# andrewdalpino/UltraZoom

Hardware: AMD Instinct MI355X
Metric: upscaled MPix/sec, MewZoom-4X 1080p bf16 batched inference (higher is better)
Workload: dtype bf16; 1 GPU; MewZoom-4X 96ch/40L bf16, 16 x 1080x1920 -> 4320x7680 per GPU; global_batch=16, parallelism=batch-sharded x1, images_in_flight=0

## Files before the change

ultrazoom_amd/csrc/mz_mix16.h:

```cpp
#pragma once
#include "mz_device.h"

namespace mz {

__device__ __forceinline__ void mix_blend_pair(float& o0, float& o1, const float b0, const float b1, const float x0, const float x1,
                                               const float z0, const float z1, const float inv_s) {
    float d0, d1;
    asm("v_mul_f32 %0, 0xbfb8aa3b, %4\n\t"
        "v_mul_f32 %1, 0xbfb8aa3b, %5\n\t"
        "v_exp_f32 %0, %0\n\t"
        "v_exp_f32 %1, %1\n\t"
        "v_fma_f32 %0, %0, %10, %10\n\t"
        "v_fma_f32 %1, %1, %10, %10\n\t"
        "v_rcp_f32 %0, %0\n\t"
        "v_rcp_f32 %1, %1\n\t"
        "v_sub_f32 %2, %8, %6\n\t"
        "v_sub_f32 %3, %9, %7\n\t"
        "v_fma_f32 %0, %0, %2, %6\n\t"
        "v_fma_f32 %1, %1, %3, %7"
        : "=&v"(o0), "=&v"(o1), "=&v"(d0), "=&v"(d1)
        : "v"(b0), "v"(b1), "v"(x0), "v"(x1), "v"(z0), "v"(z1), "s"(inv_s));
}

struct MixFrag {
    u32x4 w[3][2];
};
template <class TT, int G>
__device__ __forceinline__ void mix16_group(f32x4 (&acc)[2][12], MixFrag& f, const u32x4 (&xb)[2], uint32_t b_addr) {
    constexpr int n = G % 6, wp = G % 3;
    if constexpr (G + 2 < 24) {
        f.w[(G + 2) % 3][0] = lds_read128<(((G + 2) / 6) * 12 + 2 * ((G + 2) % 6)) * 1024>(b_addr);
        f.w[(G + 2) % 3][1] = lds_read128<(((G + 2) / 6) * 12 + 2 * ((G + 2) % 6) + 1) * 1024>(b_addr);
    }
    __builtin_amdgcn_sched_barrier(0);
    constexpr int p0 = G & 1, p1 = p0 ^ 1;
    mma16<TT>(acc[p0][2 * n], f.w[wp][0], xb[p0]);
    mma16<TT>(acc[p0][2 * n + 1], f.w[wp][1], xb[p0]);
    mma16<TT>(acc[p1][2 * n + 1], f.w[wp][1], xb[p1]);
    mma16<TT>(acc[p1][2 * n], f.w[wp][0], xb[p1]);
    __builtin_amdgcn_sched_barrier(0);
    if constexpr (G + 1 < 24) wait_w16<(G + 2 < 24 ? 2 : 0)>(f.w[(G + 1) % 3][0], f.w[(G + 1) % 3][1]);
}
template <class TT, int KS> __device__ __forceinline__ void mix16_kstep(f32x4 (&acc)[2][12], MixFrag& f, const u32x4 (&xb)[2], uint32_t b_addr) {
    mix16_group<TT, KS * 6 + 0>(acc, f, xb, b_addr);
    mix16_group<TT, KS * 6 + 1>(acc, f, xb, b_addr);
    mix16_group<TT, KS * 6 + 2>(acc, f, xb, b_addr);
    mix16_group<TT, KS * 6 + 3>(acc, f, xb, b_addr);
    mix16_group<TT, KS * 6 + 4>(acc, f, xb, b_addr);
    mix16_group<TT, KS * 6 + 5>(acc, f, xb, b_addr);
}

template <class TT>
__global__ __launch_bounds__(576) void mix16_kernel(const ConvArgs a) {
    constexpr int STAGE = 4 * 12 * 1024;
    extern __shared__ __attribute__((aligned(16))) char smem[];
    const int tid = threadIdx.x;
    const int lane = tid & 63;
    const int w = __builtin_amdgcn_readfirstlane(tid >> 6);
    int mtile, ntile;
    if (!map_tile(a, mtile, ntile)) return;
    const int nsteps = a.nchunks16;
    const int nstages = nsteps >> 2;

    if (w == 8) {
        const char* src = (const char*)a.wpk16 + (size_t)ntile * nsteps * (12 * 1024) + lane * 16;
        auto issue = [&](int st) __attribute__((always_inline)) {
            char* dst = smem + (st & 1) * STAGE;
#pragma unroll
            for (int j = 0; j < 48; ++j) glds16(src + (size_t)st * STAGE + j * 1024, dst + j * 1024);
        };
        issue(0);
        for (int st = 0; st < nstages; ++st) {
            wait_vmcnt<0>();
            __builtin_amdgcn_s_barrier();
            if (st + 1 < nstages) issue(st + 1);
        }
        return;
    }

    const int g = lane >> 4, c = lane & 15;
    const long long hw = (long long)a.Ho * a.Wo;
    const long long M = (long long)a.B * hw;
    const int half_steps = nsteps >> 1;
    const uint32_t tensor_bytes = (uint32_t)((long long)a.B * a.p0 * hw * 16);
    const __amdgpu_buffer_rsrc_t xr = __builtin_amdgcn_make_buffer_rsrc((void*)a.in0, 0, (int)tensor_bytes, 0x00020000);
    const __amdgpu_buffer_rsrc_t zr = __builtin_amdgcn_make_buffer_rsrc((void*)a.in1, 0, (int)tensor_bytes, 0x00020000);
    uint32_t voff[2];
    uint32_t vpix[2];
#pragma unroll
    for (int pf = 0; pf < 2; ++pf) {
        const long long m = (long long)mtile * 256 + 32 * w + 16 * pf + c;
        const bool in = m < M;
        const long long mm = in ? m : 0;
        const int bimg = (int)(mm / hw);
        const long long pix = mm - (long long)bimg * hw;
        vpix[pf] = in ? (uint32_t)((((long long)bimg * a.p0) * hw + pix) * 16) : 0xffffffffu;
        voff[pf] = in ? (uint32_t)((((long long)bimg * a.p0 + g) * hw + pix) * 16) : 0xffffffffu;
    }
    const uint32_t step_bytes = (uint32_t)(4 * hw * 16);
    auto load_b = [&](int ks, u32x4 (&xb)[2]) __attribute__((always_inline)) {
        const bool isz = ks >= half_steps;
        const int kk = ks >= nsteps ? 0 : (isz ? ks - half_steps : ks);
        const int so = __builtin_amdgcn_readfirstlane((int)(kk * step_bytes));
#pragma unroll
        for (int pf = 0; pf < 2; ++pf)
            xb[pf] = isz ? __builtin_amdgcn_raw_buffer_load_b128(zr, (int)voff[pf], so, 0)
                         : __builtin_amdgcn_raw_buffer_load_b128(xr, (int)voff[pf], so, 0);
    };
    f32x4 acc[2][12];
#pragma unroll
    for (int pf = 0; pf < 2; ++pf)
#pragma unroll
        for (int nf = 0; nf < 12; ++nf) acc[pf][nf] = f32x4{0.f, 0.f, 0.f, 0.f};
    const uint32_t lds_base = (uint32_t)(uintptr_t)(__attribute__((address_space(3))) char*)smem;
    const uint32_t b_lane = lds_base + lane * 16;
    u32x4 xb0[2], xb1[2], xb2[2];
    load_b(0, xb0);
    load_b(1, xb1);
    MixFrag f;
    auto stage_head = [&](uint32_t b_addr) __attribute__((always_inline)) {
        __builtin_amdgcn_s_barrier();
        f.w[0][0] = lds_read128<0>(b_addr);
        f.w[0][1] = lds_read128<1024>(b_addr);
        f.w[1][0] = lds_read128<2048>(b_addr);
        f.w[1][1] = lds_read128<3072>(b_addr);
        wait_w16<2>(f.w[0][0], f.w[0][1]);
    };
    for (int st = 0; st < nstages; st += 3) {
        const int ks = 4 * st;
        uint32_t b_addr = b_lane + (st & 1) * STAGE;
        stage_head(b_addr);
        load_b(ks + 2, xb2);  mix16_kstep<TT, 0>(acc, f, xb0, b_addr);
        load_b(ks + 3, xb0);  mix16_kstep<TT, 1>(acc, f, xb1, b_addr);
        load_b(ks + 4, xb1);  mix16_kstep<TT, 2>(acc, f, xb2, b_addr);
        load_b(ks + 5, xb2);  mix16_kstep<TT, 3>(acc, f, xb0, b_addr);
        b_addr = b_lane + ((st + 1) & 1) * STAGE;
        stage_head(b_addr);
        load_b(ks + 6, xb0);  mix16_kstep<TT, 0>(acc, f, xb1, b_addr);
        load_b(ks + 7, xb1);  mix16_kstep<TT, 1>(acc, f, xb2, b_addr);
        load_b(ks + 8, xb2);  mix16_kstep<TT, 2>(acc, f, xb0, b_addr);
        load_b(ks + 9, xb0);  mix16_kstep<TT, 3>(acc, f, xb1, b_addr);
        b_addr = b_lane + (st & 1) * STAGE;
        stage_head(b_addr);
        load_b(ks + 10, xb1); mix16_kstep<TT, 0>(acc, f, xb2, b_addr);
        load_b(ks + 11, xb2); mix16_kstep<TT, 1>(acc, f, xb0, b_addr);
        load_b(ks + 12, xb0); mix16_kstep<TT, 2>(acc, f, xb1, b_addr);
        load_b(ks + 13, xb1); mix16_kstep<TT, 3>(acc, f, xb2, b_addr);
    }
    const int nbase = ntile * 192;
    const uint32_t plane_bytes = (uint32_t)(hw * 16);
    typedef uint32_t u32x2_ __attribute__((ext_vector_type(2)));
    struct XZ { u32x2_ x[2], z[2]; };
    auto request = [&](int i, XZ& q) __attribute__((always_inline)) {
        const int pf = i / 6, n = i - 6 * pf;
        const bool in = vpix[pf] != 0xffffffffu;
#pragma unroll
        for (int k = 0; k < 2; ++k) {
            const int nf = 2 * n + k;
            const int plane = (nbase >> 3) + 2 * nf + (g >> 1);
            const uint32_t off = in ? vpix[pf] + (uint32_t)plane * plane_bytes + (g & 1) * 8 : 0xffffffffu;
            q.x[k] = __builtin_amdgcn_raw_buffer_load_b64(xr, (int)off, 0, 0);
            q.z[k] = __builtin_amdgcn_raw_buffer_load_b64(zr, (int)off, 0, 0);
        }
    };
    auto finish = [&](int i, const XZ& q) __attribute__((always_inline)) {
        const int pf = i / 6, n = i - 6 * pf;
        const bool in = vpix[pf] != 0xffffffffu;
        float v[8];
#pragma unroll
        for (int k = 0; k < 2; ++k) {
            const int nf = 2 * n + k;
            float xv[4], zv[4];
            unpack2<TT>(q.x[k][0], xv[0], xv[1]); unpack2<TT>(q.x[k][1], xv[2], xv[3]);
            unpack2<TT>(q.z[k][0], zv[0], zv[1]); unpack2<TT>(q.z[k][1], zv[2], zv[3]);
            float o0, o1, o2, o3;
            mix_blend_pair(o0, o1, acc[pf][nf][0], acc[pf][nf][1], xv[0], xv[1], zv[0], zv[1], a.inv_mix_scale);
            mix_blend_pair(o2, o3, acc[pf][nf][2], acc[pf][nf][3], xv[2], xv[3], zv[2], zv[3], a.inv_mix_scale);
            acc[pf][nf] = f32x4{o0, o1, o2, o3};
        }
#pragma unroll
        for (int j = 0; j < 4; ++j) {
            const float ea = acc[pf][2 * n][j], eb = acc[pf][2 * n + 1][j];
            const auto sw = __builtin_amdgcn_permlane16_swap(__builtin_bit_cast(uint32_t, ea), __builtin_bit_cast(uint32_t, eb), false, false);
            const uint32_t s0 = sw[0], s1 = sw[1];
            v[j] = __builtin_bit_cast(float, s0);
            v[4 + j] = __builtin_bit_cast(float, s1);
        }
        const int cu = 2 * (2 * n + (g & 1)) + (g >> 1);
        if (in) st_unit<TT>((char*)a.out + vpix[pf] + (long long)((nbase >> 3) + cu) * plane_bytes, v);
    };
    XZ qa, qb;
    request(0, qa);
#pragma unroll
    for (int i = 0; i < 12; i += 2) {
        request(i + 1, qb);
        __builtin_amdgcn_sched_barrier(0);
        finish(i, qa);
        if (i + 2 < 12) request(i + 2, qa);
        __builtin_amdgcn_sched_barrier(0);
        finish(i + 1, qb);
    }
}

template <class TT>
__global__ __launch_bounds__(512) void mix16b_kernel(const ConvArgs a) {
    constexpr int STAGE = 4 * 12 * 1024;
    extern __shared__ __attribute__((aligned(16))) char smem[];
    const int tid = threadIdx.x;
    const int lane = tid & 63;
    const int w = __builtin_amdgcn_readfirstlane(tid >> 6);
    {
        const char* wsrc = (const char*)a.wpk16 + lane * 16 + w * (18 * 1024);
        char* dst = smem + w * (18 * 1024);
#pragma unroll
        for (int j = 0; j < 18; ++j) glds16(wsrc + j * 1024, dst + j * 1024);
    }
    const int g = lane >> 4, c = lane & 15;
    const long long hw = (long long)a.Ho * a.Wo;
    const long long M = (long long)a.B * hw;
    const uint32_t tensor_bytes = (uint32_t)((long long)a.B * a.p0 * hw * 16);
    const __amdgpu_buffer_rsrc_t xr = __builtin_amdgcn_make_buffer_rsrc((void*)a.in0, 0, (int)tensor_bytes, 0x00020000);
    const __amdgpu_buffer_rsrc_t zr = __builtin_amdgcn_make_buffer_rsrc((void*)a.in1, 0, (int)tensor_bytes, 0x00020000);
    const __amdgpu_buffer_rsrc_t orr = __builtin_amdgcn_make_buffer_rsrc((void*)a.out, 0, (int)tensor_bytes, 0x00020000);
    const uint32_t step_bytes = (uint32_t)(4 * hw * 16);
    const float inv_hw = 1.0f / (float)hw;
    const int hwi = (int)hw, Mi = (int)M;
    auto offsets = [&](int u, uint32_t (&vo)[2]) __attribute__((always_inline)) {
#pragma unroll
        for (int pf = 0; pf < 2; ++pf) {
            const int m = u * 32 + 16 * pf + c;
            const bool in = m < Mi;
            const int mm = in ? m : 0;
            int bimg = (int)((float)mm * inv_hw);
            int pix = mm - bimg * hwi;
            if (pix < 0) { bimg -= 1; pix += hwi; }
            if (pix >= hwi) { bimg += 1; pix -= hwi; }
            vo[pf] = in ? ((uint32_t)(bimg * a.p0 + g) * (uint32_t)hwi + (uint32_t)pix) * 16u : 0xffffffffu;
        }
    };
    const int nunits = (Mi + 31) / 32;
    const int stride = (int)gridDim.x * 8;
    int u = (int)blockIdx.x * 8 + w;
    uint32_t voff[2];
    offsets(u, voff);
    u32x4 R[12][2];
#pragma unroll
    for (int i = 0; i < 6; ++i) {
        const int so = __builtin_amdgcn_readfirstlane((int)(i * step_bytes));
#pragma unroll
        for (int pf = 0; pf < 2; ++pf) R[i][pf] = __builtin_amdgcn_raw_buffer_load_b128(xr, (int)voff[pf], so, 0);
    }
#pragma unroll
    for (int i = 0; i < 6; ++i) {
        const int so = __builtin_amdgcn_readfirstlane((int)(i * step_bytes));
#pragma unroll
        for (int pf = 0; pf < 2; ++pf) R[6 + i][pf] = __builtin_amdgcn_raw_buffer_load_b128(zr, (int)voff[pf], so, 0);
    }
    __builtin_amdgcn_sched_barrier(0);
    wait_vmcnt<0>();
    __builtin_amdgcn_s_barrier();
    const uint32_t lds_base = (uint32_t)(uintptr_t)(__attribute__((address_space(3))) char*)smem;
    const uint32_t b_lane = lds_base + lane * 16;
    MixFrag f;
    auto stage_head = [&](uint32_t b_addr) __attribute__((always_inline)) {
        f.w[0][0] = lds_read128<0>(b_addr);
        f.w[0][1] = lds_read128<1024>(b_addr);
        f.w[1][0] = lds_read128<2048>(b_addr);
        f.w[1][1] = lds_read128<3072>(b_addr);
        wait_w16<2>(f.w[0][0], f.w[0][1]);
    };
    while (u < nunits) {
        const int un = u + stride;
        uint32_t vnext[2];
        offsets(un, vnext);
        __builtin_amdgcn_sched_barrier(0);
        f32x4 acc[2][12];
#pragma unroll
        for (int pf = 0; pf < 2; ++pf)
#pragma unroll
            for (int nf = 0; nf < 12; ++nf) acc[pf][nf] = f32x4{0.f, 0.f, 0.f, 0.f};
        stage_head(b_lane);
        mix16_kstep<TT, 0>(acc, f, R[0], b_lane);
        mix16_kstep<TT, 1>(acc, f, R[1], b_lane);
        mix16_kstep<TT, 2>(acc, f, R[2], b_lane);
        mix16_kstep<TT, 3>(acc, f, R[3], b_lane);
        stage_head(b_lane + STAGE);
        mix16_kstep<TT, 0>(acc, f, R[4], b_lane + STAGE);
        mix16_kstep<TT, 1>(acc, f, R[5], b_lane + STAGE);
        mix16_kstep<TT, 2>(acc, f, R[6], b_lane + STAGE);
        mix16_kstep<TT, 3>(acc, f, R[7], b_lane + STAGE);
        stage_head(b_lane + 2 * STAGE);
        mix16_kstep<TT, 0>(acc, f, R[8], b_lane + 2 * STAGE);
        mix16_kstep<TT, 1>(acc, f, R[9], b_lane + 2 * STAGE);
        mix16_kstep<TT, 2>(acc, f, R[10], b_lane + 2 * STAGE);
        mix16_kstep<TT, 3>(acc, f, R[11], b_lane + 2 * STAGE);
#pragma unroll
        for (int m = 0; m < 6; ++m) {
            const int so = __builtin_amdgcn_readfirstlane((int)(m * step_bytes));
#pragma unroll
            for (int pf = 0; pf < 2; ++pf) {
                float v[8];
#pragma unroll
                for (int q = 0; q < 4; ++q) {
                    float xl, xh, zl, zh;
                    unpack2<TT>(R[m][pf][q], xl, xh);
                    unpack2<TT>(R[6 + m][pf][q], zl, zh);
                    mix_blend_pair(v[2 * q], v[2 * q + 1], acc[pf][2 * m + (q >> 1)][2 * (q & 1)], acc[pf][2 * m + (q >> 1)][2 * (q & 1) + 1], xl, xh, zl, zh,
                                   a.inv_mix_scale);
                }
                u32x4 t;
                if constexpr (TT::IS_BF16) {
                    t[0] = pack_bf16(v[0], v[1]); t[1] = pack_bf16(v[2], v[3]); t[2] = pack_bf16(v[4], v[5]); t[3] = pack_bf16(v[6], v[7]);
                } else {
                    t[0] = pack_f16(v[0], v[1]); t[1] = pack_f16(v[2], v[3]); t[2] = pack_f16(v[4], v[5]); t[3] = pack_f16(v[6], v[7]);
                }
                store16_soff(t, orr, (int)voff[pf], so);
            }
#pragma unroll
            for (int pf = 0; pf < 2; ++pf) {
                R[m][pf] = __builtin_amdgcn_raw_buffer_load_b128(xr, (int)vnext[pf], so, 0);
                R[6 + m][pf] = __builtin_amdgcn_raw_buffer_load_b128(zr, (int)vnext[pf], so, 0);
            }
            __builtin_amdgcn_sched_barrier(0);
        }
        u = un;
        voff[0] = vnext[0];
        voff[1] = vnext[1];
    }
}

}
```

ultrazoom_amd/csrc/mz_mix16.hip:

```cpp
#include "mz_mix16.h"

namespace mz {

hipError_t launch_mix16(int dtype, const ConvArgs& a, hipStream_t s) {
    if (!walk_ok(a)) return hipErrorInvalidValue;
    if (a.nchunks16 <= 0 || a.nchunks16 % 12) return hipErrorInvalidValue;
    const size_t lds = 2 * 4 * 12 * 1024;
    switch (dtype) {
        case DT_BF16: return launch_lds<mix16_kernel<TBF16>>(a.grid, 576, lds, a, s);
        case DT_F16: return launch_lds<mix16_kernel<TF16>>(a.grid, 576, lds, a, s);
        default: return hipErrorInvalidValue;
    }
}

hipError_t launch_mix16b(int dtype, const ConvArgs& a, hipStream_t s, int workgroups) {
    if (a.mtiles <= 0 || a.ntiles != 1 || workgroups <= 0) return hipErrorInvalidValue;
    if (a.nchunks16 != 12) return hipErrorInvalidValue;
    const size_t lds = 3 * 4 * 12 * 1024;
    const int grid = a.mtiles < workgroups ? a.mtiles : workgroups;
    switch (dtype) {
        case DT_BF16: return launch_lds<mix16b_kernel<TBF16>>(grid, 512, lds, a, s);
        case DT_F16: return launch_lds<mix16b_kernel<TF16>>(grid, 512, lds, a, s);
        default: return hipErrorInvalidValue;
    }
}

}
```

Before: 708.6 MPix/s.

## Restructure mix16 kernel: drop producer wave, stash operand tiles for epilogue blend

Removes the dedicated producer wave. All 8 compute waves now issue their share of the weight global-to-LDS copies, double-buffered in smaller stages with explicit vmcnt waits. While the main loop streams the x/z activation tiles, the tile this block's output channels correspond to is kept: x goes to an LDS stash and z stays in registers. The epilogue then blends from these instead of re-reading x and z from global memory, and stores with packed 16-byte stores. It uses more LDS, adds registers for the kept z tiles, and adds inline-asm branches and a remapped weight row layout. It also restricts nchunks16 to 12*ntiles.

Result: no change. 710.3 MPix/s (median of 6 runs) (+0.2%).

```diff
diff --git a/ultrazoom_amd/csrc/mz_mix16.h b/ultrazoom_amd/csrc/mz_mix16.h
--- a/ultrazoom_amd/csrc/mz_mix16.h
+++ b/ultrazoom_amd/csrc/mz_mix16.h
@@ -1,5 +1,8 @@
 #pragma once
+#include <type_traits>
+
 #include "mz_device.h"
+#include "mz_mix16_rows.h"
 
 namespace mz {
 
@@ -25,10 +28,10 @@
 struct MixFrag {
     u32x4 w[3][2];
 };
-template <class TT, int G>
+template <class TT, int G, int NG = 24>
 __device__ __forceinline__ void mix16_group(f32x4 (&acc)[2][12], MixFrag& f, const u32x4 (&xb)[2], uint32_t b_addr) {
     constexpr int n = G % 6, wp = G % 3;
-    if constexpr (G + 2 < 24) {
+    if constexpr (G + 2 < NG) {
         f.w[(G + 2) % 3][0] = lds_read128<(((G + 2) / 6) * 12 + 2 * ((G + 2) % 6)) * 1024>(b_addr);
         f.w[(G + 2) % 3][1] = lds_read128<(((G + 2) / 6) * 12 + 2 * ((G + 2) % 6) + 1) * 1024>(b_addr);
     }
@@ -39,20 +42,64 @@
     mma16<TT>(acc[p1][2 * n + 1], f.w[wp][1], xb[p1]);
     mma16<TT>(acc[p1][2 * n], f.w[wp][0], xb[p1]);
     __builtin_amdgcn_sched_barrier(0);
-    if constexpr (G + 1 < 24) wait_w16<(G + 2 < 24 ? 2 : 0)>(f.w[(G + 1) % 3][0], f.w[(G + 1) % 3][1]);
-}
-template <class TT, int KS> __device__ __forceinline__ void mix16_kstep(f32x4 (&acc)[2][12], MixFrag& f, const u32x4 (&xb)[2], uint32_t b_addr) {
-    mix16_group<TT, KS * 6 + 0>(acc, f, xb, b_addr);
-    mix16_group<TT, KS * 6 + 1>(acc, f, xb, b_addr);
-    mix16_group<TT, KS * 6 + 2>(acc, f, xb, b_addr);
-    mix16_group<TT, KS * 6 + 3>(acc, f, xb, b_addr);
-    mix16_group<TT, KS * 6 + 4>(acc, f, xb, b_addr);
-    mix16_group<TT, KS * 6 + 5>(acc, f, xb, b_addr);
+    if constexpr (G + 1 < NG) wait_w16<(G + 2 < NG ? 2 : 0)>(f.w[(G + 1) % 3][0], f.w[(G + 1) % 3][1]);
+}
+template <class TT, int KS, int NG = 24>
+__device__ __forceinline__ void mix16_kstep(f32x4 (&acc)[2][12], MixFrag& f, const u32x4 (&xb)[2], uint32_t b_addr) {
+    mix16_group<TT, KS * 6 + 0, NG>(acc, f, xb, b_addr);
+    mix16_group<TT, KS * 6 + 1, NG>(acc, f, xb, b_addr);
+    mix16_group<TT, KS * 6 + 2, NG>(acc, f, xb, b_addr);
+    mix16_group<TT, KS * 6 + 3, NG>(acc, f, xb, b_addr);
+    mix16_group<TT, KS * 6 + 4, NG>(acc, f, xb, b_addr);
+    mix16_group<TT, KS * 6 + 5, NG>(acc, f, xb, b_addr);
+}
+
+template <int OFF> __device__ __forceinline__ void lds_write128(uint32_t addr, const u32x4& v) {
+    static_assert(OFF >= 0 && OFF < 65536, "ds offset is 16 bits");
+    asm volatile("ds_write_b128 %0, %1 offset:%2" ::"v"(addr), "v"(v), "n"(OFF) : "memory");
+}
+
+__device__ __forceinline__ void keep16_if_eq(u32x4& kept, const u32x4& v, int a, int b) {
+    uint32_t k0 = kept[0], k1 = kept[1], k2 = kept[2], k3 = kept[3];
+    const uint32_t v0 = v[0], v1 = v[1], v2 = v[2], v3 = v[3];
+    asm volatile("s_cmp_lg_u32 %8, %9\n\t"
+                 "s_cbranch_scc1 .Lmix16_keep_%=\n\t"
+                 "v_mov_b32 %0, %4\n\t"
+                 "v_mov_b32 %1, %5\n\t"
+                 "v_mov_b32 %2, %6\n\t"
+                 "v_mov_b32 %3, %7\n"
+                 ".Lmix16_keep_%=:"
+                 : "+v"(k0), "+v"(k1), "+v"(k2), "+v"(k3)
+                 : "v"(v0), "v"(v1), "v"(v2), "v"(v3), "s"(__builtin_amdgcn_readfirstlane(a)), "s"(__builtin_amdgcn_readfirstlane(b))
+                 : "scc");
+    kept = u32x4{k0, k1, k2, k3};
+}
+
+__device__ __forceinline__ void glds16_hidden(uint32_t voffset, const void* sbase, uint32_t lds_wave_base) {
+    asm volatile("s_mov_b32 m0, %2\n\t"
+                 "s_nop 0\n\t"
+                 "global_load_lds_dwordx4 %0, %1"
+                 :: "v"(voffset), "s"(sbase), "s"(__builtin_amdgcn_readfirstlane(lds_wave_base)) : "memory");
+}
+__device__ __forceinline__ void buf_load16_hidden(u32x4& dst, const u32x4 rsrc, uint32_t voffset, int soffset) {
+    asm volatile("buffer_load_dwordx4 %0, %1, %2, %3 offen" : "=&v"(dst) : "v"(voffset), "s"(rsrc), "s"(soffset) : "memory");
+}
+template <int N> __device__ __forceinline__ void wait_b16(u32x4& b0, u32x4& b1) {
+    asm volatile("s_waitcnt vmcnt(%2)" : "+v"(b0), "+v"(b1) : "n"(N) : "memory");
+}
+__device__ __forceinline__ void wait_b16_7_or_4(u32x4& b0, u32x4& b1, int more) {
+    asm volatile("s_cmp_lg_u32 %2, 0\n\t"
+                 "s_cbranch_scc1 .Lmix16_wait7_%=\n\t"
+                 "s_waitcnt vmcnt(4)\n"
+                 ".Lmix16_wait7_%=:\n\t"
+                 "s_waitcnt vmcnt(7)"
+                 : "+v"(b0), "+v"(b1) : "s"(__builtin_amdgcn_readfirstlane(more)) : "memory", "scc");
 }
 
 template <class TT>
-__global__ __launch_bounds__(576) void mix16_kernel(const ConvArgs a) {
-    constexpr int STAGE = 4 * 12 * 1024;
+__global__ __launch_bounds__(512) void mix16_kernel(const ConvArgs a) {
+    constexpr int STAGE = 2 * 12 * 1024;
+    constexpr int STASH = 2 * STAGE;
     extern __shared__ __attribute__((aligned(16))) char smem[];
     const int tid = threadIdx.x;
     const int lane = tid & 63;
@@ -60,33 +107,31 @@
     int mtile, ntile;
     if (!map_tile(a, mtile, ntile)) return;
     const int nsteps = a.nchunks16;
-    const int nstages = nsteps >> 2;
-
-    if (w == 8) {
-        const char* src = (const char*)a.wpk16 + (size_t)ntile * nsteps * (12 * 1024) + lane * 16;
-        auto issue = [&](int st) __attribute__((always_inline)) {
-            char* dst = smem + (st & 1) * STAGE;
-#pragma unroll
-            for (int j = 0; j < 48; ++j) glds16(src + (size_t)st * STAGE + j * 1024, dst + j * 1024);
-        };
-        issue(0);
-        for (int st = 0; st < nstages; ++st) {
-            wait_vmcnt<0>();
-            __builtin_amdgcn_s_barrier();
-            if (st + 1 < nstages) issue(st + 1);
-        }
-        return;
-    }
+    const int nstages = nsteps >> 1;
+
+    const char* wsrc = (const char*)a.wpk16 + (size_t)ntile * nsteps * (12 * 1024);
+    uint32_t wlane[3];
+#pragma unroll
+    for (int i = 0; i < 3; ++i) {
+        const int j = 3 * w + i;
+        wlane[i] = (uint32_t)((j / 12) * (12 * 1024) + mix16_rows_src(j % 12, lane));
+    }
+    const uint32_t lds_base = (uint32_t)(uintptr_t)(__attribute__((address_space(3))) char*)smem;
+    auto issue = [&](int st) __attribute__((always_inline)) {
+        const uint32_t dst = lds_base + (st & 1) * STAGE + w * (3 * 1024);
+        const uint32_t so = (uint32_t)st * STAGE;
+#pragma unroll
+        for (int i = 0; i < 3; ++i) glds16_hidden(wlane[i] + so, wsrc, dst + i * 1024);
+    };
+    issue(0);
 
     const int g = lane >> 4, c = lane & 15;
     const long long hw = (long long)a.Ho * a.Wo;
     const long long M = (long long)a.B * hw;
     const int half_steps = nsteps >> 1;
     const uint32_t tensor_bytes = (uint32_t)((long long)a.B * a.p0 * hw * 16);
-    const __amdgpu_buffer_rsrc_t xr = __builtin_amdgcn_make_buffer_rsrc((void*)a.in0, 0, (int)tensor_bytes, 0x00020000);
-    const __amdgpu_buffer_rsrc_t zr = __builtin_amdgcn_make_buffer_rsrc((void*)a.in1, 0, (int)tensor_bytes, 0x00020000);
+    const __amdgpu_buffer_rsrc_t orr = __builtin_amdgcn_make_buffer_rsrc((void*)a.out, 0, (int)tensor_bytes, 0x00020000);
     uint32_t voff[2];
-    uint32_t vpix[2];
 #pragma unroll
     for (int pf = 0; pf < 2; ++pf) {
         const long long m = (long long)mtile * 256 + 32 * w + 16 * pf + c;
@@ -94,111 +139,115 @@
         const long long mm = in ? m : 0;
         const int bimg = (int)(mm / hw);
         const long long pix = mm - (long long)bimg * hw;
-        vpix[pf] = in ? (uint32_t)((((long long)bimg * a.p0) * hw + pix) * 16) : 0xffffffffu;
         voff[pf] = in ? (uint32_t)((((long long)bimg * a.p0 + g) * hw + pix) * 16) : 0xffffffffu;
     }
     const uint32_t step_bytes = (uint32_t)(4 * hw * 16);
+    const uint64_t xbase = (uint64_t)(uintptr_t)a.in0, zbase = (uint64_t)(uintptr_t)a.in1;
     auto load_b = [&](int ks, u32x4 (&xb)[2]) __attribute__((always_inline)) {
         const bool isz = ks >= half_steps;
-        const int kk = ks >= nsteps ? 0 : (isz ? ks - half_steps : ks);
+        const bool past = ks >= nsteps;
+        const int kk = past ? 0 : (isz ? ks - half_steps : ks);
         const int so = __builtin_amdgcn_readfirstlane((int)(kk * step_bytes));
-#pragma unroll
-        for (int pf = 0; pf < 2; ++pf)
-            xb[pf] = isz ? __builtin_amdgcn_raw_buffer_load_b128(zr, (int)voff[pf], so, 0)
-                         : __builtin_amdgcn_raw_buffer_load_b128(xr, (int)voff[pf], so, 0);
+        const uint64_t base = isz ? zbase : xbase;
+        u32x4 r;
+        r[0] = __builtin_amdgcn_readfirstlane((uint32_t)base);
+        r[1] = __builtin_amdgcn_readfirstlane((uint32_t)(base >> 32) & 0xffffu);
+        r[2] = __builtin_amdgcn_readfirstlane(past ? 0u : tensor_bytes);
+        r[3] = 0x00020000u;
+#pragma unroll
+        for (int pf = 0; pf < 2; ++pf) buf_load16_hidden(xb[pf], r, voff[pf], so);
     };
     f32x4 acc[2][12];
 #pragma unroll
     for (int pf = 0; pf < 2; ++pf)
 #pragma unroll
         for (int nf = 0; nf < 12; ++nf) acc[pf][nf] = f32x4{0.f, 0.f, 0.f, 0.f};
-    const uint32_t lds_base = (uint32_t)(uintptr_t)(__attribute__((address_space(3))) char*)smem;
     const uint32_t b_lane = lds_base + lane * 16;
+    const uint32_t stash = lds_base + STASH + w * (12 * 1024) + lane * 16;
     u32x4 xb0[2], xb1[2], xb2[2];
     load_b(0, xb0);
     load_b(1, xb1);
+    u32x4 zk[6][2];
+#pragma unroll
+    for (int m = 0; m < 6; ++m)
+#pragma unroll
+        for (int pf = 0; pf < 2; ++pf) zk[m][pf] = u32x4{0u, 0u, 0u, 0u};
     MixFrag f;
+    int st = 0;
     auto stage_head = [&](uint32_t b_addr) __attribute__((always_inline)) {
+        wait_vmcnt<4>();
         __builtin_amdgcn_s_barrier();
+        if (st + 1 < nstages) issue(st + 1);
         f.w[0][0] = lds_read128<0>(b_addr);
         f.w[0][1] = lds_read128<1024>(b_addr);
         f.w[1][0] = lds_read128<2048>(b_addr);
         f.w[1][1] = lds_read128<3072>(b_addr);
         wait_w16<2>(f.w[0][0], f.w[0][1]);
     };
-    for (int st = 0; st < nstages; st += 3) {
-        const int ks = 4 * st;
+    const int own_x = 6 * ntile, own_z = half_steps + 6 * ntile;
+    for (int ks = 0; ks < nsteps; ks += 6) {
+        const bool keep_x = ks == own_x;
+        const int more = ks + 6 < nsteps;
+        auto step = [&](auto K, u32x4 (&cur)[2], u32x4 (&nxt)[2], uint32_t b_addr) __attribute__((always_inline)) {
+            constexpr int k = decltype(K)::value;
+            load_b(ks + k + 2, nxt);
+            if constexpr (k < 4) wait_b16<7>(cur[0], cur[1]);
+            else wait_b16_7_or_4(cur[0], cur[1], more);
+            if (keep_x) {
+                lds_write128<(2 * k) * 1024>(stash, cur[0]);
+                lds_write128<(2 * k + 1) * 1024>(stash, cur[1]);
+            }
+            keep16_if_eq(zk[k][0], cur[0], ks, own_z);
+            keep16_if_eq(zk[k][1], cur[1], ks, own_z);
+            mix16_kstep<TT, k & 1, 12>(acc, f, cur, b_addr);
+        };
         uint32_t b_addr = b_lane + (st & 1) * STAGE;
         stage_head(b_addr);
-        load_b(ks + 2, xb2);  mix16_kstep<TT, 0>(acc, f, xb0, b_addr);
-        load_b(ks + 3, xb0);  mix16_kstep<TT, 1>(acc, f, xb1, b_addr);
-        load_b(ks + 4, xb1);  mix16_kstep<TT, 2>(acc, f, xb2, b_addr);
-        load_b(ks + 5, xb2);  mix16_kstep<TT, 3>(acc, f, xb0, b_addr);
-        b_addr = b_lane + ((st + 1) & 1) * STAGE;
-        stage_head(b_addr);
-        load_b(ks + 6, xb0);  mix16_kstep<TT, 0>(acc, f, xb1, b_addr);
-        load_b(ks + 7, xb1);  mix16_kstep<TT, 1>(acc, f, xb2, b_addr);
-        load_b(ks + 8, xb2);  mix16_kstep<TT, 2>(acc, f, xb0, b_addr);
-        load_b(ks + 9, xb0);  mix16_kstep<TT, 3>(acc, f, xb1, b_addr);
+        step(std::integral_constant<int, 0>{}, xb0, xb2, b_addr);
+        step(std::integral_constant<int, 1>{}, xb1, xb0, b_addr);
+        ++st;
         b_addr = b_lane + (st & 1) * STAGE;
         stage_head(b_addr);
-        load_b(ks + 10, xb1); mix16_kstep<TT, 0>(acc, f, xb2, b_addr);
-        load_b(ks + 11, xb2); mix16_kstep<TT, 1>(acc, f, xb0, b_addr);
-        load_b(ks + 12, xb0); mix16_kstep<TT, 2>(acc, f, xb1, b_addr);
-        load_b(ks + 13, xb1); mix16_kstep<TT, 3>(acc, f, xb2, b_addr);
-    }
-    const int nbase = ntile * 192;
-    const uint32_t plane_bytes = (uint32_t)(hw * 16);
-    typedef uint32_t u32x2_ __attribute__((ext_vector_type(2)));
-    struct XZ { u32x2_ x[2], z[2]; };
-    auto request = [&](int i, XZ& q) __attribute__((always_inline)) {
-        const int pf = i / 6, n = i - 6 * pf;
-        const bool in = vpix[pf] != 0xffffffffu;
-#pragma unroll
-        for (int k = 0; k < 2; ++k) {
-            const int nf = 2 * n + k;
-            const int plane = (nbase >> 3) + 2 * nf + (g >> 1);
-            const uint32_t off = in ? vpix[pf] + (uint32_t)plane * plane_bytes + (g & 1) * 8 : 0xffffffffu;
-            q.x[k] = __builtin_amdgcn_raw_buffer_load_b64(xr, (int)off, 0, 0);
-            q.z[k] = __builtin_amdgcn_raw_buffer_load_b64(zr, (int)off, 0, 0);
-        }
-    };
-    auto finish = [&](int i, const XZ& q) __attribute__((always_inline)) {
-        const int pf = i / 6, n = i - 6 * pf;
-        const bool in = vpix[pf] != 0xffffffffu;
+        step(std::integral_constant<int, 2>{}, xb2, xb1, b_addr);
+        step(std::integral_constant<int, 3>{}, xb0, xb2, b_addr);
+        ++st;
+        b_addr = b_lane + (st & 1) * STAGE;
+        stage_head(b_addr);
+        step(std::integral_constant<int, 4>{}, xb1, xb0, b_addr);
+        step(std::integral_constant<int, 5>{}, xb2, xb1, b_addr);
+        ++st;
+    }
+    wait_b16<0>(xb0[0], xb0[1]);
+    wait_b16<0>(xb1[0], xb1[1]);
+    u32x4 xs[2];
+    xs[0] = lds_read128<0>(stash);
+#pragma unroll
+    for (int e = 0; e < 12; ++e) {
+        const int m = e >> 1, pf = e & 1;
+        u32x4& xe = xs[e & 1];
+        if (e + 1 < 12) {
+            xs[(e + 1) & 1] = lds_read128<0>(stash + (e + 1) * 1024);
+            asm volatile("s_waitcnt lgkmcnt(1)" : "+v"(xe)::"memory");
+        } else {
+            asm volatile("s_waitcnt lgkmcnt(0)" : "+v"(xe)::"memory");
+        }
+        const int so = __builtin_amdgcn_readfirstlane((int)((uint32_t)(6 * ntile + m) * step_bytes));
         float v[8];
 #pragma unroll
-        for (int k = 0; k < 2; ++k) {
-            const int nf = 2 * n + k;
-            float xv[4], zv[4];
-            unpack2<TT>(q.x[k][0], xv[0], xv[1]); unpack2<TT>(q.x[k][1], xv[2], xv[3]);
-            unpack2<TT>(q.z[k][0], zv[0], zv[1]); unpack2<TT>(q.z[k][1], zv[2], zv[3]);
-            float o0, o1, o2, o3;
-            mix_blend_pair(o0, o1, acc[pf][nf][0], acc[pf][nf][1], xv[0], xv[1], zv[0], zv[1], a.inv_mix_scale);
-            mix_blend_pair(o2, o3, acc[pf][nf][2], acc[pf][nf][3], xv[2], xv[3], zv[2], zv[3], a.inv_mix_scale);
-            acc[pf][nf] = f32x4{o0, o1, o2, o3};
-        }
-#pragma unroll
-        for (int j = 0; j < 4; ++j) {
-            const float ea = acc[pf][2 * n][j], eb = acc[pf][2 * n + 1][j];
-            const auto sw = __builtin_amdgcn_permlane16_swap(__builtin_bit_cast(uint32_t, ea), __builtin_bit_cast(uint32_t, eb), false, false);
-            const uint32_t s0 = sw[0], s1 = sw[1];
-            v[j] = __builtin_bit_cast(float, s0);
-            v[4 + j] = __builtin_bit_cast(float, s1);
-        }
-        const int cu = 2 * (2 * n + (g & 1)) + (g >> 1);
-        if (in) st_unit<TT>((char*)a.out + vpix[pf] + (long long)((nbase >> 3) + cu) * plane_bytes, v);
-    };
-    XZ qa, qb;
-    request(0, qa);
-#pragma unroll
-    for (int i = 0; i < 12; i += 2) {
-        request(i + 1, qb);
-        __builtin_amdgcn_sched_barrier(0);
-        finish(i, qa);
-        if (i + 2 < 12) request(i + 2, qa);
-        __builtin_amdgcn_sched_barrier(0);
-        finish(i + 1, qb);
+        for (int q = 0; q < 4; ++q) {
+            float xl, xh, zl, zh;
+            unpack2<TT>(xe[q], xl, xh);
+            unpack2<TT>(zk[m][pf][q], zl, zh);
+            mix_blend_pair(v[2 * q], v[2 * q + 1], acc[pf][2 * m + (q >> 1)][2 * (q & 1)], acc[pf][2 * m + (q >> 1)][2 * (q & 1) + 1], xl, xh, zl, zh,
+                           a.inv_mix_scale);
+        }
+        u32x4 t;
+        if constexpr (TT::IS_BF16) {
+            t[0] = pack_bf16(v[0], v[1]); t[1] = pack_bf16(v[2], v[3]); t[2] = pack_bf16(v[4], v[5]); t[3] = pack_bf16(v[6], v[7]);
+        } else {
+            t[0] = pack_f16(v[0], v[1]); t[1] = pack_f16(v[2], v[3]); t[2] = pack_f16(v[4], v[5]); t[3] = pack_f16(v[6], v[7]);
+        }
+        store16_soff(t, orr, (int)voff[pf], so);
     }
 }
 
diff --git a/ultrazoom_amd/csrc/mz_mix16.hip b/ultrazoom_amd/csrc/mz_mix16.hip
--- a/ultrazoom_amd/csrc/mz_mix16.hip
+++ b/ultrazoom_amd/csrc/mz_mix16.hip
@@ -4,11 +4,11 @@
 
 hipError_t launch_mix16(int dtype, const ConvArgs& a, hipStream_t s) {
     if (!walk_ok(a)) return hipErrorInvalidValue;
-    if (a.nchunks16 <= 0 || a.nchunks16 % 12) return hipErrorInvalidValue;
-    const size_t lds = 2 * 4 * 12 * 1024;
+    if (a.nchunks16 <= 0 || a.nchunks16 != 12 * a.ntiles) return hipErrorInvalidValue;
+    const size_t lds = (2 * 2 * 12 + 8 * 12) * 1024;
     switch (dtype) {
-        case DT_BF16: return launch_lds<mix16_kernel<TBF16>>(a.grid, 576, lds, a, s);
-        case DT_F16: return launch_lds<mix16_kernel<TF16>>(a.grid, 576, lds, a, s);
+        case DT_BF16: return launch_lds<mix16_kernel<TBF16>>(a.grid, 512, lds, a, s);
+        case DT_F16: return launch_lds<mix16_kernel<TF16>>(a.grid, 512, lds, a, s);
         default: return hipErrorInvalidValue;
     }
 }
diff --git a/ultrazoom_amd/csrc/mz_mix16_rows.h b/ultrazoom_amd/csrc/mz_mix16_rows.h
--- /dev/null
+++ b/ultrazoom_amd/csrc/mz_mix16_rows.h
@@ -0,0 +1,15 @@
+#pragma once
+
+namespace mz {
+
+constexpr int mix16_rows_channel(int frag, int row) {
+    return 32 * (frag >> 1) + 8 * (row >> 2) + 4 * (frag & 1) + (row & 3);
+}
+constexpr int mix16_rows_src(int frag, int lane) {
+    const int g = lane >> 4, c = lane & 15;
+    const int piece = 2 * (frag >> 1) + (c >> 3);
+    const int pos = g * 16 + 8 * ((c >> 2) & 1) + 4 * (frag & 1) + (c & 3);
+    return piece * 1024 + pos * 16;
+}
+
+}
```
